# 18281818221/kalle-audio

Hardware: AMD Instinct MI355X
Metric: audio-seconds/sec (node) DiT train step, 10s@12.5Hz x1024 latents (higher is better)
Workload: dtype bf16; 1 GPU; DiT train step (fwd+bwd+allreduce+Adam), 24 blocks D=1536 h=24, 10 s @ 12.5 Hz x 1024 latents (T=125+1 prepend), S=130 x 768 cross-attn cond; DiT shape chosen by this build (reference defines none); global_batch=256, per_gpu_batch=256, parallelism=dp1, objective=v, io_channels=1024, global_cond_type=prepend

## Files before the change

kalle_audio_amd/csrc/attention.hip:

```cpp
#include "common.h"
#include "../../include/kalle_hip.h"

namespace {

template <int DH>
struct Hd {
    static_assert(DH == 32 || DH == 64 || DH == 128, "head dim 32, 64 or 128");
    static constexpr int STRIDE = 2 * DH + 32;
    static constexpr int TILE = 128 * STRIDE;
    static constexpr float SCALE = DH == 32 ? 0.17677669529663687f : DH == 64 ? 0.125f : 0.08838834764831845f;
    static constexpr float SCALE_LOG2E = SCALE * 1.4426950408889634f;
    static constexpr int PAIRS = DH / 16;
    static constexpr int PAIRS_LOG2 = DH == 32 ? 1 : DH == 64 ? 2 : 3;
    static constexpr int NP = DH == 128 ? 2 : 1;
};
constexpr int AT_STRIDE = Hd<64>::STRIDE;
constexpr int AT_TILE = Hd<64>::TILE;
constexpr float SM_SCALE = Hd<64>::SCALE;
constexpr float NEG_BIG = -1.0e30f;
constexpr float SM_SCALE_LOG2E = Hd<64>::SCALE_LOG2E;
constexpr float LOG2E = 1.4426950408889634f;
constexpr float M_INIT = -2.0e30f;

template <int NT, int DH = 64>
// ... 134 lines not shown
}
__device__ __forceinline__ bf16x8 pack_pair(const f32x4& a, const f32x4& b) {
    i32x4 w;
    w[0] = (int)pack_bf16x2(a[0], a[1]);
    w[1] = (int)pack_bf16x2(a[2], a[3]);
    w[2] = (int)pack_bf16x2(b[0], b[1]);
    w[3] = (int)pack_bf16x2(b[2], b[3]);
    return __builtin_bit_cast(bf16x8, w);
}
__device__ __forceinline__ float xor16_32_max(float v) {
    v = fmaxf(v, __shfl_xor(v, 16, 64));
    return fmaxf(v, __shfl_xor(v, 32, 64));
}
__device__ __forceinline__ float xor16_32_sum(float v) {
    v += __shfl_xor(v, 16, 64);
    return v + __shfl_xor(v, 32, 64);
}

typedef float f32x2 __attribute__((ext_vector_type(2)));
__device__ __forceinline__ void mfma_results_ready() {
    __builtin_amdgcn_sched_barrier(0);
    asm volatile("s_nop 15\n\ts_nop 3" ::: "memory");
    __builtin_amdgcn_sched_barrier(0);
}
__device__ __forceinline__ float max3_raw(float a, float b, float c) {
    float r;
    asm("v_max3_f32 %0, %1, %2, %3" : "=v"(r) : "v"(a), "v"(b), "v"(c));
    return r;
}
__device__ __forceinline__ float min_raw(float a, float b) {
    float r;
    asm("v_min_f32 %0, %1, %2" : "=v"(r) : "v"(a), "v"(b));
    return r;
}
__device__ __forceinline__ f32x2 pk_add(f32x2 a, f32x2 b) {
    f32x2 r;
    asm("v_pk_add_f32 %0, %1, %2" : "=v"(r) : "v"(a), "v"(b));
    return r;
}
__device__ __forceinline__ f32x2 pk_mul(f32x2 a, f32x2 b) {
    f32x2 r;
    asm("v_pk_mul_f32 %0, %1, %2" : "=v"(r) : "v"(a), "v"(b));
    return r;
}
__device__ __forceinline__ f32x2 pk_fma(f32x2 a, f32x2 b, f32x2 c) {
    f32x2 r;
    asm("v_pk_fma_f32 %0, %1, %2, %3" : "=v"(r) : "v"(a), "v"(b), "v"(c));
    return r;
}
__device__ __forceinline__ f32x2 lo2(const f32x4& v) { return f32x2{v[0], v[1]}; }
__device__ __forceinline__ f32x2 hi2(const f32x4& v) { return f32x2{v[2], v[3]}; }

struct AttnParams {
    const bf16_t* q; int64_t ldq; int q_off;
    const bf16_t* k; int64_t ldk; int k_off;
    const bf16_t* v; int64_t ldv; int v_off;
    bf16_t* out; int64_t ldo;
    float* lse;
    const float* cosT; const float* sinT; int rot;
    const uint8_t* mask;
    int B, H, Hkv, Nq, Nk;
    int causal;
    int qpos;
    const bf16_t* dout; float* delta;
    bf16_t* dq; bf16_t* dk; bf16_t* dv;
    unsigned long long* stamps;
};
__host__ __device__ __forceinline__ bool attn_fold_tail(const AttnParams& p) {
    return !p.causal && p.rot == 0 && p.Nk > 128 && p.Nk <= 160;
}
__device__ __forceinline__ void attn_stamp(const AttnParams& p, int tid, int idx) {
    if (p.stamps && tid == 0)
        p.stamps[((int64_t)blockIdx.z * gridDim.y + blockIdx.y) * 8 + idx] = __builtin_amdgcn_s_memrealtime();
}

template <int DH>
__device__ __forceinline__ void store_row(bf16_t* row, const f32x4 (&v)[DH / 16], int g) {
    constexpr int NB = DH / 16;
    uint32_t w[NB][2];
#pragma unroll
    for (int dt = 0; dt < NB; ++dt) { w[dt][0] = pack_bf16x2(v[dt][0], v[dt][1]); w[dt][1] = pack_bf16x2(v[dt][2], v[dt][3]); }
#pragma unroll
    for (int pr = 0; pr < NB / 2; ++pr) {
        const auto a = __builtin_amdgcn_permlane16_swap(w[2 * pr][0], w[2 * pr + 1][0], false, false);
        const auto c = __builtin_amdgcn_permlane16_swap(w[2 * pr][1], w[2 * pr + 1][1], false, false);
        *reinterpret_cast<i32x4*>(row + 16 * (2 * pr + (g & 1)) + 4 * (g & ~1)) = i32x4{(int)a[0], (int)c[0], (int)a[1], (int)c[1]};
    }
}
__device__ __forceinline__ void store_row64(bf16_t* row, const f32x4& v0, const f32x4& v1, const f32x4& v2, const f32x4& v3, int g) {
    const f32x4 v[4] = {v0, v1, v2, v3};
    uint32_t w[4][2];
#pragma unroll
    for (int dt = 0; dt < 4; ++dt) { w[dt][0] = pack_bf16x2(v[dt][0], v[dt][1]); w[dt][1] = pack_bf16x2(v[dt][2], v[dt][3]); }
#pragma unroll
    for (int pr = 0; pr < 2; ++pr) {
        const auto a = __builtin_amdgcn_permlane16_swap(w[2 * pr][0], w[2 * pr + 1][0], false, false);
        const auto c = __builtin_amdgcn_permlane16_swap(w[2 * pr][1], w[2 * pr + 1][1], false, false);
        *reinterpret_cast<i32x4*>(row + 16 * (2 * pr + (g & 1)) + 4 * (g & ~1)) = i32x4{(int)a[0], (int)c[0], (int)a[1], (int)c[1]};
    }
}


template <int QT, int DH = 64>
__global__ __launch_bounds__(128 / (16 * QT) * 64, DH == 128 ? 2 : QT == 1 ? 4 : 2) void attn_fwd_kernel(AttnParams p) {
    constexpr int NT = 128 / (16 * QT) * 64;
    constexpr int STRIDE = Hd<DH>::STRIDE, TILE = Hd<DH>::TILE, KS = DH / 32, DT = DH / 16;
    constexpr float SCALE = Hd<DH>::SCALE, SCALE_LOG2E = Hd<DH>::SCALE_LOG2E;
    extern __shared__ __attribute__((aligned(16))) char smem[];
    char* Qs = smem;
    char* Ks = smem + TILE;
    char* Vs = smem + 2 * TILE;
    float* kbias = reinterpret_cast<float*>(smem + 3 * TILE);
    char* Kt = smem + 3 * TILE + 640;
    char* Vt = Kt + 32 * STRIDE;

    const int tid = threadIdx.x, lane = tid & 63, wave = tid >> 6;
    const int g = lane >> 4, li = lane & 15;
    const int b = blockIdx.z, h = blockIdx.y, q0 = (p.causal ? (int)(gridDim.x - 1 - blockIdx.x) : (int)blockIdx.x) * 128;
    const bool fold_tail = QT == 1 && attn_fold_tail(p);
    attn_stamp(p, tid, 0);
    const int hk = h / (p.H / p.Hkv);

    const bf16_t* qsrc = p.q + (int64_t)b * p.Nq * p.ldq + p.q_off + h * DH;
    const bf16_t* ksrc = p.k + (int64_t)b * p.Nk * p.ldk + p.k_off + hk * DH;
    const bf16_t* vsrc = p.v + (int64_t)b * p.Nk * p.ldv + p.v_off + hk * DH;

    {
        TileRegs<NT, DH> tq, tk, tv;
        const int kv0 = min(128, p.Nk);
        tile_load<NT, DH>(tq, qsrc, p.ldq, q0, min(128, p.Nq - q0), p.rot, tid);
        tile_load<NT, DH>(tk, ksrc, p.ldk, 0, kv0, p.rot, tid);
        tile_load<NT, DH>(tv, vsrc, p.ldv, 0, kv0, 0, tid);
        const RopeSet<DH> rq = rope_load<DH>(p.cosT, p.sinT, q0, min(128, p.Nq - q0), p.rot, tid, p.qpos);
        const RopeSet<DH> rk = rope_load<DH>(p.cosT, p.sinT, 0, kv0, p.rot, tid);
        constexpr int TCH = DH / 8, TCH_LOG2 = DH == 32 ? 2 : DH == 64 ? 3 : 4, TN = (64 * TCH + NT - 1) / NT;
        constexpr bool TEXACT = TN * NT == 64 * TCH;
        i32x4 tt[TN];
        tt[0] = i32x4{0, 0, 0, 0};
        if constexpr (TN == 2) tt[1] = i32x4{0, 0, 0, 0};
        if constexpr (QT == 1) {
            if (fold_tail) {
                auto tail_load = [&](int i) {
                    const int c = tid + NT * i;
                    const int row = (c >> TCH_LOG2) & 31, key = 128 + row;
                    if ((TEXACT || c < 64 * TCH) && key < p.Nk)
                        tt[i] = *reinterpret_cast<const i32x4*>((c < 32 * TCH ? ksrc + (int64_t)key * p.ldk : vsrc + (int64_t)key * p.ldv) +
                                                                8 * (c & (TCH - 1)));
                };
                tail_load(0);
                if constexpr (TN == 2) tail_load(1);
            }
        }
        tile_store<NT, DH>(Qs, tq, q0, min(128, p.Nq - q0), p.cosT, p.sinT, p.rot, tid, p.qpos, p.rot != 0, rq);
        tile_store<NT, DH>(Ks, tk, 0, kv0, p.cosT, p.sinT, p.rot, tid, 0, p.rot != 0, rk);
        tile_store<NT, DH>(Vs, tv, 0, kv0, nullptr, nullptr, 0, tid);
        if constexpr (QT == 1) {
            if (fold_tail) {
                auto tail_store = [&](int i) {
                    const int c = tid + NT * i;
                    if (TEXACT || c < 64 * TCH)
                        *reinterpret_cast<i32x4*>((c < 32 * TCH ? Kt : Vt) + ((c >> TCH_LOG2) & 31) * STRIDE + 16 * (c & (TCH - 1))) = tt[i];
                };
                tail_store(0);
                if constexpr (TN == 2) tail_store(1);
                if (tid < 32) {
                    float bias = 0.f;
                    if (128 + tid >= p.Nk) bias = -INFINITY;
                    else if (p.mask && !p.mask[(int64_t)b * p.Nk + 128 + tid]) bias = NEG_BIG;
                    kbias[128 + tid] = bias;
                }
            }
        }
    }
    __syncthreads();
    attn_stamp(p, tid, 1);
    bf16x8 qf[QT][KS];
#pragma unroll
    for (int qt = 0; qt < QT; ++qt)
#pragma unroll
        for (int s = 0; s < KS; ++s) qf[qt][s] = rowfrag<DH>(Qs, wave * (16 * QT) + 16 * qt, s, lane);

// ... 1572 lines not shown
```

kalle_audio_amd/csrc/common.h:

```cpp
#pragma once
#include <hip/hip_runtime.h>
#include <stdint.h>

#include <atomic>

#define KALLE_OK 0
#define KALLE_ERR_ARG -1
#define KALLE_ERR_LAUNCH -2
#define KALLE_ERR_UNSUPPORTED -3

typedef __attribute__((ext_vector_type(8))) __bf16 bf16x8;
typedef __attribute__((ext_vector_type(4))) __bf16 bf16x4;
typedef __attribute__((ext_vector_type(2))) __bf16 bf16x2;
typedef __attribute__((ext_vector_type(4))) short s16x4;
typedef __attribute__((ext_vector_type(8))) short s16x8;
typedef __attribute__((ext_vector_type(4))) float f32x4;
typedef __attribute__((ext_vector_type(2))) float f32x2;
typedef __attribute__((ext_vector_type(4))) int i32x4;
typedef __attribute__((ext_vector_type(2))) int i32x2;
typedef unsigned short bf16_t;

#define LDS_PTR(T, p) ((__attribute__((address_space(3))) T*)(p))

__device__ __forceinline__ float bf16_to_f32(bf16_t v) {
    return __builtin_bit_cast(float, ((uint32_t)v) << 16);
}
__device__ __forceinline__ bf16_t f32_to_bf16(float f) {
    __bf16 b = (__bf16)f;
    return __builtin_bit_cast(bf16_t, b);
}
__device__ __forceinline__ uint32_t pack_bf16x2(float lo, float hi) {
    bf16x2 v;
    v[0] = (__bf16)lo;
    v[1] = (__bf16)hi;
    return __builtin_bit_cast(uint32_t, v);
}
__device__ __forceinline__ float bf16lo(uint32_t w) { return __builtin_bit_cast(float, w << 16); }
__device__ __forceinline__ float bf16hi(uint32_t w) { return __builtin_bit_cast(float, w & 0xffff0000u); }

__device__ __forceinline__ float wave_sum(float v) {
#pragma unroll
    for (int o = 32; o > 0; o >>= 1) v += __shfl_xor(v, o, 64);
    return v;
}
__device__ __forceinline__ float wave_max(float v) {
#pragma unroll
    for (int o = 32; o > 0; o >>= 1) v = fmaxf(v, __shfl_xor(v, o, 64));
    return v;
}

__device__ __forceinline__ float block_sum(float v, float* red) {
    v = wave_sum(v);
    const int lane = threadIdx.x & 63, w = threadIdx.x >> 6, nw = (blockDim.x + 63) >> 6;
    __syncthreads();
    if (lane == 0) red[w] = v;
    __syncthreads();
    float t = 0.f;
    for (int i = 0; i < nw; ++i) t += red[i];
    return t;
}

__device__ __forceinline__ float sigmoidf_(float x) { return 1.f / (1.f + __expf(-x)); }
__device__ __forceinline__ float siluf_(float x) { return x * sigmoidf_(x); }

__device__ __forceinline__ __amdgpu_buffer_rsrc_t make_rsrc(const void* p, uint32_t bytes) {
    return __builtin_amdgcn_make_buffer_rsrc((void*)p, 0, bytes, 0x00020000);
}

#define KALLE_LAUNCH(...)            \
    do {                             \
        (void)hipGetLastError();     \
        hipLaunchKernelGGL(__VA_ARGS__); \
    } while (0)

static inline void kalle_allow_lds(const void* kernel, int bytes, std::atomic<uint64_t>& done) {
    int dev = 0;
    (void)hipGetDevice(&dev);
    const uint64_t bit = 1ull << (dev & 63);
    if (done.load(std::memory_order_relaxed) & bit) return;
    (void)hipFuncSetAttribute(kernel, hipFuncAttributeMaxDynamicSharedMemorySize, bytes);
    done.fetch_or(bit, std::memory_order_relaxed);
}

extern "C" void kalle_set_last_error(const char* what);
static inline int kalle_check_launch() {
    hipError_t e = hipGetLastError();
    if (e == hipSuccess) return KALLE_OK;
    kalle_set_last_error(hipGetErrorName(e));
    return KALLE_ERR_LAUNCH;
}
```

kalle_audio_amd/csrc/gemm2.hip:

```cpp
#include <stdio.h>
#include <stdlib.h>
#include <string.h>

#include <algorithm>
#include <functional>
#include <type_traits>
#include <utility>

#include "gemm_common.h"
#include "../../include/kalle_hip.h"

namespace {

constexpr int BK2 = 64;
#define GPTR(p) ((const __attribute__((address_space(1))) void*)(p))

__device__ __attribute__((aligned(64))) const unsigned kalle_zero_block[16] = {0, 0, 0, 0, 0, 0, 0, 0, 0, 0, 0, 0, 0, 0, 0, 0};

template <bool KM, int R, int NW>
struct Loader {
    static constexpr int PER_WAVE = (R / 8) / NW;
    const bf16_t* src[PER_WAVE];
    int64_t kstep;

// ... 271 lines not shown
                        sg[2 * e] += bf16lo((uint32_t)og[e]); sg[2 * e + 1] += bf16hi((uint32_t)og[e]);
                    }
                    bf16_t* dp = reinterpret_cast<bf16_t*>(p.C) + (int64_t)gm * p.ldc;
                    *reinterpret_cast<i32x4*>(dp + j0) = ox;
                    *reinterpret_cast<i32x4*>(dp + p.glu_inner + j0) = og;
                }
            }
        } else if (p.atomic) {
            const int gn = col0 + lane;
#pragma unroll 4
            for (int r = 0; r < 16; ++r) {
                const int gm = rbase + r;
                if (gm < p.M && gn < p.N)
                    atomicAdd(reinterpret_cast<float*>(p.C) + (int64_t)gm * p.ldc + gn, patch[pidx(r, lane)] * p.alpha);
            }
        } else if constexpr (C_F32) {
#pragma unroll
            for (int i = 0; i < 4; ++i) {
                const int r = g + 4 * i;
                const int gm = rbase + r, gn = col0 + 4 * li;
                if (gm >= p.M || gn >= p.N) continue;
                const f32x4 pv = *reinterpret_cast<const f32x4*>(patch + pidx(r, 4 * li));
                float v[4] = {pv[0], pv[1], pv[2], pv[3]};
                const int64_t crow = gemm_crow(p, gm);
                gemm_epilogue4(p, gm, gn, crow, v, false, &bias4);
                if (pre_res) {
#pragma unroll
                    for (int j = 0; j < 4; ++j) v[j] += rcur[i][j];
                }
                float* cp = reinterpret_cast<float*>(p.C) + crow * p.ldc + gn;
                if (p.accumulate) {
                    const f32x4 c0 = *reinterpret_cast<const f32x4*>(cp);
#pragma unroll
                    for (int j = 0; j < 4; ++j) v[j] += c0[j];
                }
                *reinterpret_cast<f32x4*>(cp) = f32x4{v[0], v[1], v[2], v[3]};
            }
        } else {
#pragma unroll
            for (int half = 0; half < 2; ++half) {
                const int r = (lane >> 3) + 8 * half;
                const int gm = rbase + r, gn = col0 + 8 * (lane & 7);
                if (gm >= p.M || gn >= p.N) continue;
                const f32x4 p0 = *reinterpret_cast<const f32x4*>(patch + pidx(r, 8 * (lane & 7)));
                const f32x4 p1 = *reinterpret_cast<const f32x4*>(patch + pidx(r, 8 * (lane & 7) + 4));
                float v0[4] = {p0[0], p0[1], p0[2], p0[3]}, v1[4] = {p1[0], p1[1], p1[2], p1[3]};
                const int64_t crow = gemm_crow(p, gm);
                gemm_epilogue4(p, gm, gn, crow, v0, true, &bias8[0]);
                gemm_epilogue4(p, gm, gn + 4, crow, v1, true, &bias8[1]);
                i32x4 o;
                o[0] = (int)pack_bf16x2(v0[0], v0[1]);
                o[1] = (int)pack_bf16x2(v0[2], v0[3]);
                o[2] = (int)pack_bf16x2(v1[0], v1[1]);
                o[3] = (int)pack_bf16x2(v1[2], v1[3]);
                *reinterpret_cast<i32x4*>(reinterpret_cast<bf16_t*>(p.C) + crow * p.ldc + gn) = o;
            }
        }
        asm volatile("s_waitcnt lgkmcnt(0)" ::: "memory");
    }
    if constexpr (GLU == 2) {
        if (p.glu_dbias) {
#pragma unroll
            for (int e = 0; e < 8; ++e) {
#pragma unroll
                for (int o = 8; o < 64; o <<= 1) { sx[e] += __shfl_xor(sx[e], o, 64); sg[e] += __shfl_xor(sg[e], o, 64); }
            }
            const int j0 = col0 + (lane & 7) * 8;
            if (lane < 8 && j0 < p.glu_inner) {
#pragma unroll
                for (int e = 0; e < 8; ++e) {
                    atomicAdd(p.glu_dbias + j0 + e, sx[e]);
                    atomicAdd(p.glu_dbias + p.glu_inner + j0 + e, sg[e]);
                }
            }
        }
    }
    if (p.stamps) {
        gemm_stamp(p, wave, lane, 4, stamp_slot);
        asm volatile("s_waitcnt vmcnt(0)" ::: "memory");
        gemm_stamp(p, wave, lane, 5, stamp_slot);
    }
}

#define MFMA16(FA, FB)                                                                                         \
    _Pragma("unroll") for (int mt = 0; mt < 4; ++mt) _Pragma("unroll") for (int nt = 0; nt < 4; ++nt)          \
        acc[mt][nt] = __builtin_amdgcn_mfma_f32_16x16x32_bf16(__builtin_bit_cast(bf16x8, FA[mt]),              \
                                                              __builtin_bit_cast(bf16x8, FB[nt]), acc[mt][nt], 0, 0, 0)

template <bool A_KM, bool B_KM, bool C_F32, int WM, int WN, int TM, int GLU = 0, int NS = 3>
__global__ __launch_bounds__(WM * WN * 64, 2) void gemm2_kernel(GemmParams p) {
    static_assert(TM == 4, "wave tile is 64 x 64");
    constexpr int TN = 4;
    constexpr int NW = WM * WN;
    constexpr int BM = WM * TM * 16, BN = WN * TN * 16;
    constexpr int A_BYTES = BM * 128, B_BYTES = BN * 128, STAGE = A_BYTES + B_BYTES;
    extern __shared__ __attribute__((aligned(16))) char smem[];
    const unsigned lds0 = (unsigned)(size_t)LDS_PTR(char, smem);

    const int tid = threadIdx.x, lane = tid & 63;
    const int wave = __builtin_amdgcn_readfirstlane(tid >> 6);
    const int wm = wave / WN, wn = wave % WN;

    int tm, tn;
    gemm_tile_coords(blockIdx.x, gridDim.x, p.tiles_m, p.tiles_n, p.group_m, tm, tn);
    const int m0 = tm * BM, n0 = tn * BN;

    const int nk_all = (p.K + BK2 - 1) / BK2;
    const int kt0 = blockIdx.y * p.ktiles_per_split;
    const int nk = min(p.ktiles_per_split, nk_all - kt0);
    const int kvalid = p.K % BK2;
    const int tail_t = kvalid ? nk_all - 1 - kt0 : -1;

    f32x4 acc[TM][TN];
#pragma unroll
    for (int i = 0; i < TM; ++i)
#pragma unroll
        for (int j = 0; j < TN; ++j) acc[i][j] = f32x4{0.f, 0.f, 0.f, 0.f};

    Loader<A_KM, BM, NW> la;
    Loader<B_KM, BN, NW> lb;
    la.init(p.A, p.lda, p.M, m0, kt0 * BK2, wave, lane);
    lb.init(p.B, p.ldb, p.N, n0, kt0 * BK2, wave, lane, GLU == 1 ? p.glu_inner : 0, tn);
    const int arow = wm * TM * 16, bcol = wn * TN * 16;
    Reader<A_KM, BM> ra;
    Reader<B_KM, BN> rb;
    ra.init(lds0, arow, lane);
    rb.init(lds0 + A_BYTES, bcol, lane);

    {
    constexpr int PT = Loader<A_KM, BM, NW>::PER_WAVE + Loader<B_KM, BN, NW>::PER_WAVE;
    static_assert((NS - 2) * PT <= 63, "vmcnt is a 6-bit counter");
    {
        const int pre = nk < NS ? nk : NS;
#pragma unroll
        for (int t = 0; t < NS; ++t) {
            if (t < pre) {
                la.issue_at(smem + t * STAGE, wave, lane, t, tail_t, kvalid);
                lb.issue_at(smem + t * STAGE + A_BYTES, wave, lane, t, tail_t, kvalid);
            }
        }
        constexpr int PRE_KEEP = (NS - 1) * PT <= 63 ? NS - 1 : NS - 2;
        const int keep = pre - 1 < PRE_KEEP ? pre - 1 : PRE_KEEP;
        auto wait_keep = [&](auto self, auto c) {
            constexpr int C = decltype(c)::value;
            if (keep == C) asm volatile("s_waitcnt vmcnt(%0)" ::"n"(C * PT) : "memory");
            if constexpr (C > 0) self(self, std::integral_constant<int, C - 1>{});
        };
        wait_keep(wait_keep, std::integral_constant<int, PRE_KEEP>{});
    }
    __builtin_amdgcn_s_barrier();
    __builtin_amdgcn_sched_barrier(0);

    i32x4 fa0[4], fb0[4], fa1[4], fb1[4];
    ra.template read<0, 4>(0, fa0);
    rb.template read<0, 4>(0, fb0);

    unsigned so_cur = 0, so_nxt = STAGE;
    int kt = 0;

    auto iteration = [&](auto issue_c, auto next_c, auto keep_c) {
        constexpr bool ISSUE = decltype(issue_c)::value, NEXT = decltype(next_c)::value;
        constexpr int KEEP = decltype(keep_c)::value;
        asm volatile("s_waitcnt lgkmcnt(0)" ::: "memory");
        __builtin_amdgcn_sched_barrier(0);
        ra.template read<1, 4>(so_cur, fa1);
        rb.template read<1, 4>(so_cur, fb1);
// ... 140 lines not shown
        so_nxt = so_nxt + STAGE >= NS * STAGE ? 0 : so_nxt + STAGE;
    };
    using T_ = std::true_type;
    using F_ = std::false_type;
    using P0 = std::integral_constant<int, 0>;
    using P1 = std::integral_constant<int, 1>;
    using KS_ = std::integral_constant<int, NS - 2>;
#pragma unroll 1
    for (; kt + NS + 1 < nk; kt += 2) {
        iteration(P0{}, T_{}, T_{}, KS_{});
        ++kt; iteration(P1{}, T_{}, T_{}, KS_{}); --kt;
    }
    int par = 0;
    if (kt + NS < nk) { iteration(P0{}, T_{}, T_{}, KS_{}); ++kt; par = 1; }
    auto tail = [&](auto self, auto r) {
        constexpr int R = decltype(r)::value;
        if (nk - 1 - kt == R) {
            if (par) iteration(P1{}, F_{}, T_{}, std::integral_constant<int, R - 1>{});
            else iteration(P0{}, F_{}, T_{}, std::integral_constant<int, R - 1>{});
            ++kt; par ^= 1;
        }
        if constexpr (R > 1) self(self, std::integral_constant<int, R - 1>{});
    };
    tail(tail, std::integral_constant<int, NS - 1>{});
    if (par) iteration(P1{}, F_{}, F_{}, P0{});
    else iteration(P0{}, F_{}, F_{}, P0{});

    asm volatile("s_waitcnt vmcnt(0) lgkmcnt(0)" ::: "memory");
    __builtin_amdgcn_s_barrier();
    float* red = reinterpret_cast<float*>(smem + RED_OFF) + wt * 4096;
    if (kg == 1) {
#pragma unroll
        for (int i = 0; i < TM; ++i)
#pragma unroll
            for (int j = 0; j < TN; ++j) *reinterpret_cast<f32x4*>(red + ((i * TN + j) * 64 + lane) * 4) = acc[i][j];
    }
    asm volatile("s_waitcnt lgkmcnt(0)" ::: "memory");
    __builtin_amdgcn_s_barrier();
    if (kg == 1) {
        __builtin_amdgcn_s_barrier();
        return;
    }
#pragma unroll
    for (int i = 0; i < TM; ++i)
#pragma unroll
        for (int j = 0; j < TN; ++j) acc[i][j] += *reinterpret_cast<const f32x4*>(red + ((i * TN + j) * 64 + lane) * 4);
    if constexpr (C_F32) {
        if (p.slab_stride) {
            GemmParams q = p;
            q.C = static_cast<float*>(p.C) + (int64_t)blockIdx.y * p.slab_stride;
            wave_epilogue<C_F32, TM>(q, acc, smem, wt, lane, m0 + arow, n0 + bcol);
            return;
        }
    }
    wave_epilogue<C_F32, TM, GLU>(p, acc, smem, wt, lane, m0 + arow, GLU == 1 ? tn * (BN / 2) + wn * 32 : n0 + bcol);
}

template <bool B_KM, bool C_F32, int WM, int WN, int GLU, int NS>
int launch2_ks2(const GemmParams& p, hipStream_t st) {
    constexpr int lds = NS * (WM + WN) * 64 * 128;
    static_assert(lds <= 160 * 1024, "LDS per workgroup");
    static std::atomic<uint64_t> lds_ok{0};
    kalle_allow_lds(reinterpret_cast<const void*>(gemm2_ks2_kernel<B_KM, C_F32, WM, WN, GLU, NS>), lds, lds_ok);
    dim3 grid(p.tiles_m * p.tiles_n, p.splits), block(WM * WN * 128);
    KALLE_LAUNCH((gemm2_ks2_kernel<B_KM, C_F32, WM, WN, GLU, NS>), grid, block, lds, st, p);
    return kalle_check_launch();
}

template <bool A_KM, bool B_KM, bool C_F32, int WM, int WN, int TM, int GLU = 0, int NS = 3>
int launch2(const GemmParams& p, hipStream_t st) {
    constexpr int BM = WM * TM * 16, BN = WN * 64;
    constexpr int lds = NS * (BM + BN) * 128;
    static_assert(lds <= 160 * 1024, "LDS per workgroup");
    static std::atomic<uint64_t> lds_ok{0};
    kalle_allow_lds(reinterpret_cast<const void*>(gemm2_kernel<A_KM, B_KM, C_F32, WM, WN, TM, GLU, NS>), lds, lds_ok);
    dim3 grid(p.tiles_m * p.tiles_n, p.splits), block(WM * WN * 64);
    KALLE_LAUNCH((gemm2_kernel<A_KM, B_KM, C_F32, WM, WN, TM, GLU, NS>), grid, block, lds, st, p);
    return kalle_check_launch();
}



constexpr int GEMM3_LDS = 2 * (256 + 256) * 128 + 8 * 16 * 64 * 4;

static int kalle_cu_count() {
    static std::atomic<int> cached[64];
    int dev = 0;
    (void)hipGetDevice(&dev);
    int v = cached[dev & 63].load(std::memory_order_relaxed);
    if (v > 0) return v;
    hipDeviceProp_t prop;
    v = hipGetDeviceProperties(&prop, dev) == hipSuccess && prop.multiProcessorCount > 0 ? prop.multiProcessorCount : 256;
    v &= ~7;
    if (v < 8) v = 8;
    cached[dev & 63].store(v, std::memory_order_relaxed);
    return v;
}

#define MFMA32(FA, FB)                                                                                         \
    _Pragma("unroll") for (int mt = 0; mt < 8; ++mt) _Pragma("unroll") for (int nt = 0; nt < 4; ++nt)          \
        acc[mt][nt] = __builtin_amdgcn_mfma_f32_16x16x32_bf16(__builtin_bit_cast(bf16x8, FA[mt]),              \
                                                              __builtin_bit_cast(bf16x8, FB[nt]), acc[mt][nt], 0, 0, 0)

constexpr int SCHED_SETS = 256;
constexpr int SCHED_LINE = 32;
__device__ int kalle_gemm_sched[SCHED_SETS][9 * SCHED_LINE];

__device__ __forceinline__ int sched_issue(int* sched, int xcd) { return atomicAdd(sched + xcd * SCHED_LINE, 1); }
__device__ __forceinline__ int sched_resolve(int xcd, int raw, int first_round, int ntiles) {
    const int id = xcd + 8 * (first_round + raw);
    return id < ntiles ? id : ntiles;
}
__device__ __forceinline__ void sched_leave(int* sched, int nwg) {
    if (atomicAdd(sched + 8 * SCHED_LINE, 1) == nwg - 1) {
#pragma unroll
        for (int i = 0; i < 9; ++i) atomicExch(sched + i * SCHED_LINE, 0);
    }
}

template <bool A_KM, bool B_KM, bool C_F32, int GLU, bool XCD_RASTER, bool PERSIST>
__device__ __forceinline__ void gemm3_tiles(const GemmParams& p, int tile0, int tstride, int tile_end, int ntiles_raster, int kt0,
                                            int nk) {
    const int kvalid = p.K % BK2;
    const int tail_t = kvalid ? (p.K + BK2 - 1) / BK2 - 1 - kt0 : -1;
    constexpr int WN = 4, TM = 8, NW = 8;
    constexpr int BM = 256, BN = 256;
    constexpr int A_BYTES = BM * 128, B_BYTES = BN * 128, STAGE = A_BYTES + B_BYTES;
    extern __shared__ __attribute__((aligned(16))) char smem[];
    const unsigned lds0 = (unsigned)(size_t)LDS_PTR(char, smem);

    const int tid = threadIdx.x, lane = tid & 63;
    const int wave = __builtin_amdgcn_readfirstlane(tid >> 6);
    const int wm = wave / WN, wn = wave % WN;
    const int arow = wm * 128, bcol = wn * 64;
    Loader<A_KM, BM, NW> la;
    Loader<B_KM, BN, NW> lb;
    Reader<A_KM, BM> ra;
    Reader<B_KM, BN> rb;
    ra.init(lds0, arow, lane);
    rb.init(lds0 + A_BYTES, bcol, lane);
    const bool late = wave >= NW / 2;
    if (late) __builtin_amdgcn_s_setprio(1);

    auto coords = [&](int tile, int& tm, int& tn) {
        if constexpr (XCD_RASTER) gemm_tile_coords(tile, ntiles_raster, p.tiles_m, p.tiles_n, p.group_m, tm, tn);
        else gemm_tile_coords_plain(tile, p.tiles_m, p.tiles_n, p.group_m, tm, tn);
    };
    auto init_loaders = [&](int tm, int tn, int kt_first) {
        la.init(p.A, p.lda, p.M, tm * BM, (kt0 + kt_first) * BK2, wave, lane);
        lb.init(p.B, p.ldb, p.N, tn * BN, (kt0 + kt_first) * BK2, wave, lane, GLU == 1 ? p.glu_inner : 0, tn);
    };
    bool prefetched = false;
    unsigned s0 = 0;

    int* const sched = PERSIST && p.sched_set > 0 ? &kalle_gemm_sched[p.sched_set - 1][0] : nullptr;
    int next_tile = tile_end;
    int drawn = 0;
    if constexpr (PERSIST) {
        if (sched && tid == 0) drawn = sched_issue(sched, blockIdx.x & 7);
    }
    volatile int* const mailbox = reinterpret_cast<volatile int*>(smem + 2 * STAGE);
    for (int tile = tile0; tile < tile_end; tile = next_tile) {
        int tm, tn;
        coords(tile, tm, tn);
        const int m0 = tm * BM, n0 = tn * BN;
        next_tile = PERSIST ? tile + tstride : tile_end;
        bool has_next = PERSIST && next_tile < tile_end;
        gemm_stamp(p, wave, lane, 0, tile);
        f32x4 acc[TM][4];
#pragma unroll
        for (int i = 0; i < TM; ++i)
#pragma unroll
            for (int j = 0; j < 4; ++j) acc[i][j] = f32x4{0.f, 0.f, 0.f, 0.f};

        if (!prefetched) {
            init_loaders(tm, tn, 0);
            la.issue_at(smem, wave, lane, 0, tail_t, kvalid);
            lb.issue_at(smem + A_BYTES, wave, lane, 0, tail_t, kvalid);
            s0 = 0;
            if (nk > 1) {
                la.issue_at(smem + STAGE, wave, lane, 1, tail_t, kvalid);
                lb.issue_at(smem + STAGE + A_BYTES, wave, lane, 1, tail_t, kvalid);
                asm volatile("s_waitcnt vmcnt(8)" ::: "memory");
            } else {
                asm volatile("s_waitcnt vmcnt(0)" ::: "memory");
            }
        } else if constexpr (PERSIST) {
            init_loaders(tm, tn, nk > 1 ? 2 : 1);
            asm volatile("s_waitcnt vmcnt(0)" ::: "memory");
        }
        if constexpr (PERSIST) {
            if (sched && tid == 0) {
                *mailbox = sched_resolve(blockIdx.x & 7, drawn, tstride >> 3, tile_end);
                asm volatile("s_waitcnt lgkmcnt(0)" ::: "memory");
            }
        }
        __builtin_amdgcn_s_barrier();
        __builtin_amdgcn_sched_barrier(0);
        if constexpr (PERSIST) {
            if (sched) {
                next_tile = __builtin_amdgcn_readfirstlane(*mailbox);
                has_next = next_tile < tile_end;
            }
        }
        gemm_stamp(p, wave, lane, 1, tile);

        i32x4 fa[8], fb[4];
        unsigned so_cur = s0;
        int kt = 0;
        ra.template read<0, 8>(so_cur, fa);
        rb.template read<0, 4>(so_cur, fb);

        auto iteration = [&](auto issue_c, auto next_c) {
            constexpr bool ISSUE = decltype(issue_c)::value, NEXT = decltype(next_c)::value;
            asm volatile("s_waitcnt lgkmcnt(0)" ::: "memory");
            __builtin_amdgcn_sched_barrier(0);
            MFMA32(fa, fb);
            __builtin_amdgcn_sched_barrier(0);
            ra.template read<1, 8>(so_cur, fa);
            rb.template read<1, 4>(so_cur, fb);
            asm volatile("s_waitcnt lgkmcnt(0)" ::: "memory");
            __builtin_amdgcn_sched_barrier(0);
            if (!late) {
                MFMA32(fa, fb);
                __builtin_amdgcn_sched_barrier(0);
            }
            asm volatile("s_waitcnt vmcnt(0)" ::: "memory");
            __builtin_amdgcn_s_barrier();
            __builtin_amdgcn_sched_barrier(0);
            if (late) {
                MFMA32(fa, fb);
                __builtin_amdgcn_sched_barrier(0);
            }
            if constexpr (ISSUE) {
                la.issue_at(smem + so_cur, wave, lane, kt + 2, tail_t, kvalid);
                lb.issue_at(smem + so_cur + A_BYTES, wave, lane, kt + 2, tail_t, kvalid);
            }
            so_cur ^= STAGE;
            if constexpr (NEXT) {
                ra.template read<0, 8>(so_cur, fa);
                rb.template read<0, 4>(so_cur, fb);
            }
            __builtin_amdgcn_sched_barrier(0);
        };
        auto last_iteration = [&]() {
            asm volatile("s_waitcnt lgkmcnt(0)" ::: "memory");
            __builtin_amdgcn_sched_barrier(0);
            MFMA32(fa, fb);
            __builtin_amdgcn_sched_barrier(0);
            ra.template read<1, 8>(so_cur, fa);
            rb.template read<1, 4>(so_cur, fb);
            asm volatile("s_waitcnt lgkmcnt(0)" ::: "memory");
            __builtin_amdgcn_sched_barrier(0);
            MFMA32(fa, fb);
            __builtin_amdgcn_sched_barrier(0);
        };
        using T_ = std::true_type;
        using F_ = std::false_type;
#pragma unroll 1
        for (; kt + 2 < nk; ++kt) iteration(T_{}, T_{});
        if (kt + 1 < nk) { iteration(F_{}, T_{}); ++kt; }
        if constexpr (!PERSIST || GLU == 2) iteration(F_{}, F_{});
        else last_iteration();
        gemm_stamp(p, wave, lane, 2, tile);

        const unsigned s_last = so_cur;
        auto hook = [&]() {
            if constexpr (!PERSIST) return;
            if (has_next) {
                int ntm, ntn;
                coords(next_tile, ntm, ntn);
                init_loaders(ntm, ntn, 0);
                la.issue_at(smem + (s_last ^ STAGE), wave, lane, 0, tail_t, kvalid);
                lb.issue_at(smem + (s_last ^ STAGE) + A_BYTES, wave, lane, 0, tail_t, kvalid);
                if (nk > 1) {
                    la.issue_at(smem + s_last, wave, lane, 1, tail_t, kvalid);
                    lb.issue_at(smem + s_last + A_BYTES, wave, lane, 1, tail_t, kvalid);
                }
                if (sched && tid == 0) drawn = sched_issue(sched, blockIdx.x & 7);
            }
        };
        wave_epilogue<C_F32, TM, GLU>(p, acc, smem + 2 * STAGE, wave, lane, m0 + arow, GLU == 1 ? tn * 128 + wn * 32 : n0 + bcol,
                                      hook, tile);
        prefetched = has_next;
        s0 = s_last ^ STAGE;
        if constexpr (!PERSIST) break;
    }
}

template <bool A_KM, bool B_KM, bool C_F32, int GLU = 0>
__global__ __launch_bounds__(512, 2) void gemm3_kernel(GemmParams p) {
    const int nk_all = (p.K + BK2 - 1) / BK2;
    const int ntiles = p.tiles_m * p.tiles_n;
    if constexpr (A_KM) {
        if (p.mix_na >= 0) {
            const int na = p.mix_na, sa = p.mix_sa;
            int bid = blockIdx.x, tile, slice, per;
            if (bid < na * sa) { tile = bid % na; slice = bid / na; per = (nk_all + sa - 1) / sa; }
            else { bid -= na * sa; const int nb = ntiles - na; tile = na + bid % nb; slice = bid / nb; per = (nk_all + sa) / (sa + 1); }
            const int kt0 = slice * per, nk = min(per, nk_all - kt0);
            if (nk <= 0) return;
            gemm3_tiles<A_KM, B_KM, C_F32, GLU, true, false>(p, tile, 0, tile + 1, ntiles, kt0, nk);
        } else {
            const int kt0 = blockIdx.y * p.ktiles_per_split;
            gemm3_tiles<A_KM, B_KM, C_F32, GLU, true, false>(p, blockIdx.x, 0, blockIdx.x + 1, ntiles, kt0,
                                                             min(p.ktiles_per_split, nk_all - kt0));
        }
    } else {
        gemm3_tiles<A_KM, B_KM, C_F32, GLU, true, true>(p, blockIdx.x, gridDim.x, ntiles, ntiles, 0, nk_all);
        if (p.sched_set > 0 && threadIdx.x == 0) sched_leave(&kalle_gemm_sched[p.sched_set - 1][0], gridDim.x);
    }
}

struct GroupProblem {
    const bf16_t* A;
    const bf16_t* B;
    float* C;
    int64_t lda, ldb, ldc;
    int M, N, K;
    int tiles_m, tiles_n, group_m;
    int unsplit, splits;
    int r1_start, r2_start;
};
struct GroupParams {
    int nprob, r2_base;
    int overwrite;
    GroupProblem pr[KALLE_MAX_GROUP];
};

__global__ __launch_bounds__(256) void gemm3_group_zero_kernel(GroupParams gp) {
    int pi = 0, base = 0;
    const int bid = blockIdx.x >> 2, band = blockIdx.x & 3;
    for (;;) {
        const int nb = gp.pr[pi].tiles_m * gp.pr[pi].tiles_n - gp.pr[pi].unsplit;
        if (bid < base + nb || pi + 1 >= gp.nprob) break;
        base += nb;
        ++pi;
    }
    const GroupProblem& q = gp.pr[pi];
    int tm, tn;
    gemm_tile_coords_plain(q.unsplit + bid - base, q.tiles_m, q.tiles_n, q.group_m, tm, tn);
    const int r0 = tm * 256 + band * 64, c0 = tn * 256;
    for (int i = threadIdx.x; i < 64 * 64; i += 256) {
        const int r = r0 + i / 64, c = c0 + (i & 63) * 4;
        if (r < q.M && c < q.N) *reinterpret_cast<f32x4*>(q.C + (int64_t)r * q.ldc + c) = f32x4{0.f, 0.f, 0.f, 0.f};
    }
}

__global__ __launch_bounds__(512, 2) void gemm3_wgrad_group_kernel(GroupParams gp) {
    const bool whole = (int)blockIdx.x < gp.r2_base;
    const int bid = whole ? xcd_contiguous(blockIdx.x, gp.r2_base)
                          : gp.r2_base + xcd_contiguous(blockIdx.x - gp.r2_base, gridDim.x - gp.r2_base);
    int pi = 0, tile, slice = 0;
    if (whole) {
        while (pi + 1 < gp.nprob && bid >= gp.pr[pi + 1].r1_start) ++pi;
        tile = bid - gp.pr[pi].r1_start;
    } else {
        while (pi + 1 < gp.nprob && bid >= gp.pr[pi + 1].r2_start) ++pi;
        const int local = bid - gp.pr[pi].r2_start, nb = gp.pr[pi].tiles_m * gp.pr[pi].tiles_n - gp.pr[pi].unsplit;
        tile = gp.pr[pi].unsplit + local % nb;
        slice = local / nb;
    }
    const GroupProblem& q = gp.pr[pi];
    GemmParams p{};
    p.A = q.A; p.B = q.B; p.C = q.C;
    p.lda = q.lda; p.ldb = q.ldb; p.ldc = q.ldc;
    p.M = q.M; p.N = q.N; p.K = q.K;
    p.alpha = 1.f;
    p.rows_per_batch = 1;
    p.accumulate = gp.overwrite ? 0 : 1;
    p.atomic = whole ? 0 : 1;
    const int ntiles = q.tiles_m * q.tiles_n, nk_all = (q.K + BK2 - 1) / BK2;
    p.tiles_m = q.tiles_m; p.tiles_n = q.tiles_n; p.group_m = q.group_m;
    int kt0 = 0, nk = nk_all;
    if (!whole) {
        const int per = (nk_all + q.splits - 1) / q.splits;
        kt0 = slice * per;
        nk = min(per, nk_all - kt0);
        if (nk <= 0) return;
    }
    gemm3_tiles<true, true, true, 0, false, false>(p, tile, 0, tile + 1, ntiles, kt0, nk);
}

template <bool A_KM, bool B_KM, bool C_F32, int GLU = 0>
int launch3(const GemmParams& p, hipStream_t st) {
    constexpr int lds = GEMM3_LDS;
    static std::atomic<uint64_t> lds_ok{0};
    kalle_allow_lds(reinterpret_cast<const void*>(gemm3_kernel<A_KM, B_KM, C_F32, GLU>), lds, lds_ok);
    dim3 grid(p.tiles_m * p.tiles_n, p.splits), block(512);
    if (p.mix_na >= 0) {
        const int ntiles = p.tiles_m * p.tiles_n;
        grid = dim3(p.mix_na * p.mix_sa + (ntiles - p.mix_na) * (p.mix_sa + 1), 1);
    } else if (!A_KM) {
        if (p.splits != 1) return KALLE_ERR_UNSUPPORTED;
        const int cus = kalle_cu_count();
        if ((int)grid.x > cus) {
            GemmParams q = p;
            grid.x = cus;
            static std::atomic<unsigned> next_set{0};
            hipStreamCaptureStatus cap = hipStreamCaptureStatusNone;
            const bool capturing = hipStreamIsCapturing(st, &cap) == hipSuccess && cap != hipStreamCaptureStatusNone;
            q.sched_set = !capturing ? 1 + (int)(next_set.fetch_add(1, std::memory_order_relaxed) % SCHED_SETS) : 0;
            KALLE_LAUNCH((gemm3_kernel<A_KM, B_KM, C_F32, GLU>), grid, block, lds, st, q);
            return kalle_check_launch();
        }
    }
    KALLE_LAUNCH((gemm3_kernel<A_KM, B_KM, C_F32, GLU>), grid, block, lds, st, p);
    return kalle_check_launch();
}

int launch3_layout(const GemmParams& p, bool a_km, bool b_km, bool f32, hipStream_t st) {
    if (!a_km && !b_km) return f32 ? launch3<false, false, true>(p, st) : launch3<false, false, false>(p, st);
    if (!a_km && b_km) return f32 ? launch3<false, true, true>(p, st) : launch3<false, true, false>(p, st);
    if (a_km && b_km) return launch3<true, true, true>(p, st);
    return KALLE_ERR_UNSUPPORTED;
}

template <int WM, int WN, int TM>
int launch2_layout(const GemmParams& p, bool a_km, bool b_km, bool f32, hipStream_t st) {
    if (!a_km && !b_km) return f32 ? launch2<false, false, true, WM, WN, TM>(p, st) : launch2<false, false, false, WM, WN, TM>(p, st);
    if (!a_km && b_km) return f32 ? launch2<false, true, true, WM, WN, TM>(p, st) : launch2<false, true, false, WM, WN, TM>(p, st);
    if (a_km && b_km) return launch2<true, true, true, WM, WN, TM>(p, st);
    return KALLE_ERR_UNSUPPORTED;
}

struct CuReplay {
    double cu[256] = {};
    void run(int tiles, int nk, int slices) {
        if (tiles <= 0 || slices <= 0) return;
        const int per = (nk + slices - 1) / slices;
        for (int sl = 0; sl < slices; ++sl) {
            const int k = nk - sl * per < per ? nk - sl * per : per;
            if (k <= 0) break;
            const double d = 10.0 + 1.6 * k;
            for (int t = 0; t < tiles; ++t) {
                std::pop_heap(cu, cu + 256, std::greater<double>());
                cu[255] += d;
                std::push_heap(cu, cu + 256, std::greater<double>());
            }
        }
    }
    double makespan() const {
        double mk = 0.0;
        for (int c = 0; c < 256; ++c) mk = cu[c] > mk ? cu[c] : mk;
        return mk;
    }
};

inline bool al16(const void* p) { return (reinterpret_cast<uintptr_t>(p) & 15) == 0; }


void fill_plan(GemmPlan& g, int family, const GemmParams& p, int bm, int bn, int splits) {
    const int nk = (p.K + BK2 - 1) / BK2;
    g.family = family;
    g.tile_n = bn;
    g.tiles_m = (p.M + bm - 1) / bm;
    g.tiles_n = (p.N + bn - 1) / bn;
    g.group_m = g.tiles_m < 4 ? g.tiles_m : 4;
    g.ktiles_per_split = (nk + splits - 1) / splits;
    g.splits = (nk + g.ktiles_per_split - 1) / g.ktiles_per_split;
}

bool plan_small_tiles(const GemmParams& p, const GemmLayout& l, const void* ws, int64_t ws_bytes, GemmPlan& g) {
    if (l.a_km || p.M > 2048 || (p.N & 63) || (l.b_km && (p.N & 127))) return false;
    if ((int64_t)((p.M + 255) / 256) * ((p.N + 255) / 256) >= 256) return false;
    const int nk = (p.K + BK2 - 1) / BK2;
    static const int cand[3][2] = {{1, 1}, {2, 1}, {2, 2}};
    int wm = 0, wn = 0, splits = 1;
    double best = 1e30;
// ... 471 lines not shown
```

Before: 11600 audio-seconds/sec.

## Write bf16 GEMM outputs directly from registers via transposed MFMA and lane swaps

For bf16-output gemm3 kernels, the MFMA operands are swapped so each lane holds a transposed accumulator fragment. A new register-direct epilogue then packs and lane-swaps (permlane16_swap, DPP) the values and stores them straight to global memory instead of staging them through LDS. This also shrinks the dynamic LDS reservation for these kernels, which can allow higher occupancy. The risks are that fused GLU forward/backward and bias paths are reimplemented with different store coalescing and extra DPP/atomic traffic; the attention change is a refactor into a shared helper.

```diff
diff --git a/kalle_audio_amd/csrc/attention.hip b/kalle_audio_amd/csrc/attention.hip
--- a/kalle_audio_amd/csrc/attention.hip
+++ b/kalle_audio_amd/csrc/attention.hip
@@ -240,9 +240,7 @@
     for (int dt = 0; dt < NB; ++dt) { w[dt][0] = pack_bf16x2(v[dt][0], v[dt][1]); w[dt][1] = pack_bf16x2(v[dt][2], v[dt][3]); }
 #pragma unroll
     for (int pr = 0; pr < NB / 2; ++pr) {
-        const auto a = __builtin_amdgcn_permlane16_swap(w[2 * pr][0], w[2 * pr + 1][0], false, false);
-        const auto c = __builtin_amdgcn_permlane16_swap(w[2 * pr][1], w[2 * pr + 1][1], false, false);
-        *reinterpret_cast<i32x4*>(row + 16 * (2 * pr + (g & 1)) + 4 * (g & ~1)) = i32x4{(int)a[0], (int)c[0], (int)a[1], (int)c[1]};
+        *reinterpret_cast<i32x4*>(row + 32 * pr + pair8_col(g)) = pair8(w[2 * pr][0], w[2 * pr][1], w[2 * pr + 1][0], w[2 * pr + 1][1]);
     }
 }
 __device__ __forceinline__ void store_row64(bf16_t* row, const f32x4& v0, const f32x4& v1, const f32x4& v2, const f32x4& v3, int g) {
@@ -252,9 +250,7 @@
     for (int dt = 0; dt < 4; ++dt) { w[dt][0] = pack_bf16x2(v[dt][0], v[dt][1]); w[dt][1] = pack_bf16x2(v[dt][2], v[dt][3]); }
 #pragma unroll
     for (int pr = 0; pr < 2; ++pr) {
-        const auto a = __builtin_amdgcn_permlane16_swap(w[2 * pr][0], w[2 * pr + 1][0], false, false);
-        const auto c = __builtin_amdgcn_permlane16_swap(w[2 * pr][1], w[2 * pr + 1][1], false, false);
-        *reinterpret_cast<i32x4*>(row + 16 * (2 * pr + (g & 1)) + 4 * (g & ~1)) = i32x4{(int)a[0], (int)c[0], (int)a[1], (int)c[1]};
+        *reinterpret_cast<i32x4*>(row + 32 * pr + pair8_col(g)) = pair8(w[2 * pr][0], w[2 * pr][1], w[2 * pr + 1][0], w[2 * pr + 1][1]);
     }
 }
 
diff --git a/kalle_audio_amd/csrc/common.h b/kalle_audio_amd/csrc/common.h
--- a/kalle_audio_amd/csrc/common.h
+++ b/kalle_audio_amd/csrc/common.h
@@ -37,6 +37,13 @@
 }
 __device__ __forceinline__ float bf16lo(uint32_t w) { return __builtin_bit_cast(float, w << 16); }
 __device__ __forceinline__ float bf16hi(uint32_t w) { return __builtin_bit_cast(float, w & 0xffff0000u); }
+
+__device__ __forceinline__ i32x4 pair8(uint32_t b0w0, uint32_t b0w1, uint32_t b1w0, uint32_t b1w1) {
+    const auto a = __builtin_amdgcn_permlane16_swap(b0w0, b1w0, false, false);
+    const auto c = __builtin_amdgcn_permlane16_swap(b0w1, b1w1, false, false);
+    return i32x4{(int)a[0], (int)c[0], (int)a[1], (int)c[1]};
+}
+__device__ __forceinline__ int pair8_col(int g) { return 16 * (g & 1) + 4 * (g & ~1); }
 
 __device__ __forceinline__ float wave_sum(float v) {
 #pragma unroll
diff --git a/kalle_audio_amd/csrc/gemm2.hip b/kalle_audio_amd/csrc/gemm2.hip
--- a/kalle_audio_amd/csrc/gemm2.hip
+++ b/kalle_audio_amd/csrc/gemm2.hip
@@ -377,6 +377,177 @@
     }
 }
 
+__device__ __forceinline__ void row_trade(const i32x4& o0, const i32x4& o1, bool hi, i32x4& ra, i32x4& rb) {
+#pragma unroll
+    for (int e = 0; e < 4; ++e) {
+        const int keep = hi ? o1[e] : o0[e], send = hi ? o0[e] : o1[e];
+        const int recv = __builtin_amdgcn_update_dpp(0, send, 0x128, 0xf, 0xf, false);
+        ra[e] = hi ? recv : keep;
+        rb[e] = hi ? keep : recv;
+    }
+}
+
+template <int TM, int GLU = 0, typename Hook = NoHook>
+__device__ __forceinline__ void wave_epilogue_direct(const GemmParams& p, f32x4 (&acc)[TM][4], int wave, int lane, int row0,
+                                                     int col0, Hook after_barrier = Hook{}, int stamp_slot = -1) {
+    const int g = lane >> 4, li = lane & 15;
+    const int c4 = 4 * g;
+    const int c8 = pair8_col(g);
+    const bool hi = li >= 8;
+    const int jt = col0 + 32 * (li >> 3) + c8;
+    i32x4 hbuf[2][2];
+    auto load_h = [&](int mt, i32x4 (&hv)[2][2]) {
+#pragma unroll
+        for (int h2 = 0; h2 < 2; ++h2) {
+            const int gm = row0 + 16 * mt + 8 * h2 + (li & 7);
+            hv[h2][0] = i32x4{0, 0, 0, 0};
+            hv[h2][1] = i32x4{0, 0, 0, 0};
+            if (gm < p.M && jt < p.glu_inner) {
+                const bf16_t* hp = static_cast<const bf16_t*>(p.glu_aux) + (int64_t)gm * 2 * p.glu_inner;
+                hv[h2][0] = *reinterpret_cast<const i32x4*>(hp + jt);
+                hv[h2][1] = *reinterpret_cast<const i32x4*>(hp + p.glu_inner + jt);
+            }
+        }
+    };
+    asm volatile("s_waitcnt lgkmcnt(0)" ::: "memory");
+    __builtin_amdgcn_s_barrier();
+    after_barrier();
+    gemm_stamp(p, wave, lane, 3, stamp_slot);
+    if constexpr (GLU == 2) load_h(0, hbuf);
+    float sx[8], sg[8];
+#pragma unroll
+    for (int e = 0; e < 8; ++e) { sx[e] = 0.f; sg[e] = 0.f; }
+    f32x4 bias[4];
+#pragma unroll
+    for (int nt = 0; nt < 4; ++nt) bias[nt] = f32x4{0.f, 0.f, 0.f, 0.f};
+    if (p.bias) {
+        if constexpr (GLU == 1) {
+#pragma unroll
+            for (int nt = 0; nt < 2; ++nt) {
+                const int j = col0 + 16 * nt + c4;
+                if (j < p.glu_inner) {
+                    bias[nt] = *reinterpret_cast<const f32x4*>(p.bias + j);
+                    bias[2 + nt] = *reinterpret_cast<const f32x4*>(p.bias + p.glu_inner + j);
+                }
+            }
+        } else if constexpr (GLU == 0) {
+#pragma unroll
+            for (int nt = 0; nt < 4; ++nt) {
+                const int gn = col0 + 16 * nt + c4;
+                if (gn < p.N) bias[nt] = *reinterpret_cast<const f32x4*>(p.bias + gn);
+            }
+        }
+    }
+#pragma unroll
+    for (int mt = 0; mt < TM; ++mt) {
+        const int gm = row0 + 16 * mt + li;
+        const bool rok = gm < p.M;
+        if constexpr (GLU == 1) {
+            uint32_t hx[2][2], hg[2][2], av[2][2];
+#pragma unroll
+            for (int nt = 0; nt < 2; ++nt)
+#pragma unroll
+                for (int e = 0; e < 2; ++e) {
+                    hx[nt][e] = pack_bf16x2(acc[mt][nt][2 * e] + bias[nt][2 * e], acc[mt][nt][2 * e + 1] + bias[nt][2 * e + 1]);
+                    hg[nt][e] = pack_bf16x2(acc[mt][2 + nt][2 * e] + bias[2 + nt][2 * e],
+                                            acc[mt][2 + nt][2 * e + 1] + bias[2 + nt][2 * e + 1]);
+                    const float x0 = bf16lo(hx[nt][e]), x1 = bf16hi(hx[nt][e]);
+                    const float g0 = bf16lo(hg[nt][e]), g1 = bf16hi(hg[nt][e]);
+                    av[nt][e] = pack_bf16x2(x0 * siluf_(g0), x1 * siluf_(g1));
+                }
+            const i32x4 ox = pair8(hx[0][0], hx[0][1], hx[1][0], hx[1][1]);
+            const i32x4 og = pair8(hg[0][0], hg[0][1], hg[1][0], hg[1][1]);
+            const i32x4 oa = pair8(av[0][0], av[0][1], av[1][0], av[1][1]);
+            const int j0 = col0 + c8;
+            if (rok && j0 < p.glu_inner) {
+                bf16_t* hp = reinterpret_cast<bf16_t*>(p.C) + (int64_t)gm * p.ldc;
+                *reinterpret_cast<i32x4*>(hp + j0) = ox;
+                *reinterpret_cast<i32x4*>(hp + p.glu_inner + j0) = og;
+                *reinterpret_cast<i32x4*>(static_cast<bf16_t*>(p.glu_aux) + (int64_t)gm * p.glu_inner + j0) = oa;
+            }
+        } else if constexpr (GLU == 2) {
+            i32x4 hcur[2][2];
+#pragma unroll
+            for (int h2 = 0; h2 < 2; ++h2) { hcur[h2][0] = hbuf[h2][0]; hcur[h2][1] = hbuf[h2][1]; }
+            if (mt + 1 < TM) load_h(mt + 1, hbuf);
+            uint32_t dw[4][2];
+#pragma unroll
+            for (int nt = 0; nt < 4; ++nt) {
+                dw[nt][0] = pack_bf16x2(acc[mt][nt][0] * p.alpha, acc[mt][nt][1] * p.alpha);
+                dw[nt][1] = pack_bf16x2(acc[mt][nt][2] * p.alpha, acc[mt][nt][3] * p.alpha);
+            }
+            i32x4 dvr[2];
+            row_trade(pair8(dw[0][0], dw[0][1], dw[1][0], dw[1][1]), pair8(dw[2][0], dw[2][1], dw[3][0], dw[3][1]), hi, dvr[0], dvr[1]);
+#pragma unroll
+            for (int h2 = 0; h2 < 2; ++h2) {
+                const int gmr = row0 + 16 * mt + 8 * h2 + (li & 7);
+                if (gmr < p.M && jt < p.glu_inner) {
+                    const i32x4 xv = hcur[h2][0], gv = hcur[h2][1], dv = dvr[h2];
+                    i32x4 ox, og;
+#pragma unroll
+                    for (int e = 0; e < 4; ++e) {
+                        const float x[2] = {bf16lo((uint32_t)xv[e]), bf16hi((uint32_t)xv[e])};
+                        const float gg[2] = {bf16lo((uint32_t)gv[e]), bf16hi((uint32_t)gv[e])};
+                        const float d[2] = {bf16lo((uint32_t)dv[e]), bf16hi((uint32_t)dv[e])};
+                        float dx[2], dg[2];
+#pragma unroll
+                        for (int q = 0; q < 2; ++q) {
+                            const float sgm = sigmoidf_(gg[q]);
+                            dx[q] = d[q] * gg[q] * sgm;
+                            dg[q] = d[q] * x[q] * sgm * (1.f + gg[q] * (1.f - sgm));
+                        }
+                        ox[e] = (int)pack_bf16x2(dx[0], dx[1]);
+                        og[e] = (int)pack_bf16x2(dg[0], dg[1]);
+                        sx[2 * e] += bf16lo((uint32_t)ox[e]); sx[2 * e + 1] += bf16hi((uint32_t)ox[e]);
+                        sg[2 * e] += bf16lo((uint32_t)og[e]); sg[2 * e + 1] += bf16hi((uint32_t)og[e]);
+                    }
+                    bf16_t* dp = reinterpret_cast<bf16_t*>(p.C) + (int64_t)gmr * p.ldc;
+                    *reinterpret_cast<i32x4*>(dp + jt) = ox;
+                    *reinterpret_cast<i32x4*>(dp + p.glu_inner + jt) = og;
+                }
+            }
+        } else {
+            const int64_t crow = rok ? gemm_crow(p, gm) : 0;
+            uint32_t w[4][2];
+#pragma unroll
+            for (int nt = 0; nt < 4; ++nt) {
+                float v[4] = {acc[mt][nt][0], acc[mt][nt][1], acc[mt][nt][2], acc[mt][nt][3]};
+                const int gn = col0 + 16 * nt + c4;
+                if (rok && gn < p.N) gemm_epilogue4(p, gm, gn, crow, v, true, &bias[nt]);
+                w[nt][0] = pack_bf16x2(v[0], v[1]);
+                w[nt][1] = pack_bf16x2(v[2], v[3]);
+            }
+#pragma unroll
+            for (int pr = 0; pr < 2; ++pr) {
+                const i32x4 o = pair8(w[2 * pr][0], w[2 * pr][1], w[2 * pr + 1][0], w[2 * pr + 1][1]);
+                const int gn = col0 + 32 * pr + c8;
+                if (rok && gn < p.N) *reinterpret_cast<i32x4*>(reinterpret_cast<bf16_t*>(p.C) + crow * p.ldc + gn) = o;
+            }
+        }
+    }
+    if constexpr (GLU == 2) {
+        if (p.glu_dbias) {
+#pragma unroll
+            for (int e = 0; e < 8; ++e) {
+#pragma unroll
+                for (int o = 1; o < 8; o <<= 1) { sx[e] += __shfl_xor(sx[e], o, 64); sg[e] += __shfl_xor(sg[e], o, 64); }
+            }
+            if ((li & 7) == 0 && jt < p.glu_inner) {
+#pragma unroll
+                for (int e = 0; e < 8; ++e) {
+                    atomicAdd(p.glu_dbias + jt + e, sx[e]);
+                    atomicAdd(p.glu_dbias + p.glu_inner + jt + e, sg[e]);
+                }
+            }
+        }
+    }
+    if (p.stamps) {
+        gemm_stamp(p, wave, lane, 4, stamp_slot);
+        asm volatile("s_waitcnt vmcnt(0)" ::: "memory");
+        gemm_stamp(p, wave, lane, 5, stamp_slot);
+    }
+}
+
 #define MFMA16(FA, FB)                                                                                         \
     _Pragma("unroll") for (int mt = 0; mt < 4; ++mt) _Pragma("unroll") for (int nt = 0; nt < 4; ++nt)          \
         acc[mt][nt] = __builtin_amdgcn_mfma_f32_16x16x32_bf16(__builtin_bit_cast(bf16x8, FA[mt]),              \
@@ -683,6 +854,7 @@
 
 
 constexpr int GEMM3_LDS = 2 * (256 + 256) * 128 + 8 * 16 * 64 * 4;
+constexpr int GEMM3_LDS_DIRECT = 2 * (256 + 256) * 128 + 128;
 
 static int kalle_cu_count() {
     static std::atomic<int> cached[64];
@@ -703,6 +875,11 @@
         acc[mt][nt] = __builtin_amdgcn_mfma_f32_16x16x32_bf16(__builtin_bit_cast(bf16x8, FA[mt]),              \
                                                               __builtin_bit_cast(bf16x8, FB[nt]), acc[mt][nt], 0, 0, 0)
 
+#define MFMA32T(FA, FB)                                                                                        \
+    _Pragma("unroll") for (int mt = 0; mt < 8; ++mt) _Pragma("unroll") for (int nt = 0; nt < 4; ++nt)          \
+        acc[mt][nt] = __builtin_amdgcn_mfma_f32_16x16x32_bf16(__builtin_bit_cast(bf16x8, FB[nt]),              \
+                                                              __builtin_bit_cast(bf16x8, FA[mt]), acc[mt][nt], 0, 0, 0)
+
 constexpr int SCHED_SETS = 256;
 constexpr int SCHED_LINE = 32;
 __device__ int kalle_gemm_sched[SCHED_SETS][9 * SCHED_LINE];
@@ -726,6 +903,7 @@
     const int tail_t = kvalid ? (p.K + BK2 - 1) / BK2 - 1 - kt0 : -1;
     constexpr int WN = 4, TM = 8, NW = 8;
     constexpr int BM = 256, BN = 256;
+    constexpr bool DIRECT = !C_F32;
     constexpr int A_BYTES = BM * 128, B_BYTES = BN * 128, STAGE = A_BYTES + B_BYTES;
     extern __shared__ __attribute__((aligned(16))) char smem[];
     const unsigned lds0 = (unsigned)(size_t)LDS_PTR(char, smem);
@@ -807,6 +985,10 @@
         gemm_stamp(p, wave, lane, 1, tile);
 
         i32x4 fa[8], fb[4];
+        auto mfma32 = [&]() {
+            if constexpr (DIRECT) { MFMA32T(fa, fb); }
+            else { MFMA32(fa, fb); }
+        };
         unsigned so_cur = s0;
         int kt = 0;
         ra.template read<0, 8>(so_cur, fa);
@@ -816,21 +998,21 @@
             constexpr bool ISSUE = decltype(issue_c)::value, NEXT = decltype(next_c)::value;
             asm volatile("s_waitcnt lgkmcnt(0)" ::: "memory");
             __builtin_amdgcn_sched_barrier(0);
-            MFMA32(fa, fb);
+            mfma32();
             __builtin_amdgcn_sched_barrier(0);
             ra.template read<1, 8>(so_cur, fa);
             rb.template read<1, 4>(so_cur, fb);
             asm volatile("s_waitcnt lgkmcnt(0)" ::: "memory");
             __builtin_amdgcn_sched_barrier(0);
             if (!late) {
-                MFMA32(fa, fb);
+                mfma32();
                 __builtin_amdgcn_sched_barrier(0);
             }
             asm volatile("s_waitcnt vmcnt(0)" ::: "memory");
             __builtin_amdgcn_s_barrier();
             __builtin_amdgcn_sched_barrier(0);
             if (late) {
-                MFMA32(fa, fb);
+                mfma32();
                 __builtin_amdgcn_sched_barrier(0);
             }
             if constexpr (ISSUE) {
@@ -847,13 +1029,13 @@
         auto last_iteration = [&]() {
             asm volatile("s_waitcnt lgkmcnt(0)" ::: "memory");
             __builtin_amdgcn_sched_barrier(0);
-            MFMA32(fa, fb);
+            mfma32();
             __builtin_amdgcn_sched_barrier(0);
             ra.template read<1, 8>(so_cur, fa);
             rb.template read<1, 4>(so_cur, fb);
             asm volatile("s_waitcnt lgkmcnt(0)" ::: "memory");
             __builtin_amdgcn_sched_barrier(0);
-            MFMA32(fa, fb);
+            mfma32();
             __builtin_amdgcn_sched_barrier(0);
         };
         using T_ = std::true_type;
@@ -881,8 +1063,11 @@
                 if (sched && tid == 0) drawn = sched_issue(sched, blockIdx.x & 7);
             }
         };
-        wave_epilogue<C_F32, TM, GLU>(p, acc, smem + 2 * STAGE, wave, lane, m0 + arow, GLU == 1 ? tn * 128 + wn * 32 : n0 + bcol,
-                                      hook, tile);
+        if constexpr (DIRECT)
+            wave_epilogue_direct<TM, GLU>(p, acc, wave, lane, m0 + arow, GLU == 1 ? tn * 128 + wn * 32 : n0 + bcol, hook, tile);
+        else
+            wave_epilogue<C_F32, TM, GLU>(p, acc, smem + 2 * STAGE, wave, lane, m0 + arow, GLU == 1 ? tn * 128 + wn * 32 : n0 + bcol,
+                                          hook, tile);
         prefetched = has_next;
         s0 = s_last ^ STAGE;
         if constexpr (!PERSIST) break;
@@ -985,7 +1170,7 @@
 
 template <bool A_KM, bool B_KM, bool C_F32, int GLU = 0>
 int launch3(const GemmParams& p, hipStream_t st) {
-    constexpr int lds = GEMM3_LDS;
+    constexpr int lds = C_F32 ? GEMM3_LDS : GEMM3_LDS_DIRECT;
     static std::atomic<uint64_t> lds_ok{0};
     kalle_allow_lds(reinterpret_cast<const void*>(gemm3_kernel<A_KM, B_KM, C_F32, GLU>), lds, lds_ok);
     dim3 grid(p.tiles_m * p.tiles_n, p.splits), block(512);
```

Result: no change. 11670 audio-seconds/sec (median of 6 runs) (+0.7%).
